# robdancer/SymbolicRegression.jl

Measured on AMD Instinct MI355X. Metric: tree-node x row evals/sec (whole node), 1k trees x 1M rows f32; % VALU peak, higher is better.
Workload: dtype f32; 1 GPU; C2 eval-only: 1024 random trees (size<=30) x 1M rows x 5 features Float32, fused L2 loss; ntrees_per_gpu=1024, rows=1000000, features=5, parallelism=single, trees_ok=808

## Files before the change

include/srhip.h:

```cpp
#ifndef SRHIP_H
#define SRHIP_H

#include <stdint.h>

#ifdef __cplusplus
extern "C" {
#endif

enum {
  SRHIP_OK = 0,
  SRHIP_ERR_INVALID = 1,
  SRHIP_ERR_UNSUPPORTED = 2,
  SRHIP_ERR_DEVICE = 3,
  SRHIP_ERR_NOMEM = 4
};

enum { SRHIP_F32 = 0, SRHIP_F64 = 1, SRHIP_I32 = 2 };

enum {
  SRHIP_OP_ADD = 1, SRHIP_OP_SUB = 2, SRHIP_OP_MUL = 3, SRHIP_OP_DIV = 4,
  SRHIP_OP_POW = 5,
  SRHIP_OP_GREATER = 6,
  SRHIP_OP_COND = 7,
  SRHIP_OP_LOGICAL_OR = 8,
// ... 152 lines not shown

typedef struct srhip_optim_options {
  int32_t iterations;
  int32_t nrestarts;
  uint64_t seed;
  double g_tol;
} srhip_optim_options;

int srhip_optimize_constants(srhip_ctx* ctx, const srhip_dataset* ds, srhip_program* prog,
                             const srhip_loss* loss, const int64_t* idx, int64_t nidx,
                             const srhip_optim_options* opt, double* out_loss,
                             uint8_t* out_improved, int64_t* out_fcalls);
int srhip_optimize_constants_starts(srhip_ctx* ctx, const srhip_dataset* ds, srhip_program* prog,
                                    const srhip_loss* loss, const int64_t* idx, int64_t nidx,
                                    const srhip_optim_options* opt, const double* starts_in,
                                    double* starts_out, double* out_loss, uint8_t* out_improved,
                                    int64_t* out_fcalls);

int srhip_eval_loss_grad_rowsets(srhip_ctx* ctx, const srhip_dataset* ds, srhip_program* prog,
                                 const srhip_loss* loss, const int64_t* row_offsets ,
                                 const int64_t* rows, double* out_loss, double* out_grad,
                                 uint8_t* out_ok);

int srhip_optimize_constants_rowsets(srhip_ctx* ctx, const srhip_dataset* ds, srhip_program* prog,
                                     const srhip_loss* loss, const int64_t* row_offsets ,
                                     const int64_t* rows, const srhip_optim_options* opt,
                                     const uint64_t* tree_seeds ,
                                     const double* starts_in , double* starts_out ,
                                     double* out_loss, uint8_t* out_improved, int64_t* out_fcalls);

double srhip_last_kernel_ms(const srhip_ctx* ctx);
int srhip_last_work(const srhip_ctx* ctx, int64_t out[4]);
int64_t srhip_hot_form_launches(const srhip_ctx* ctx);
int srhip_program_stats(const srhip_program* prog, int64_t* total_nodes, int64_t* total_opnodes,
                        int32_t* max_stack);
int srhip_program_derived(const srhip_program* prog, int32_t* count, uint32_t* spec, int32_t cap);
int32_t srhip_isa_handler_count(void);
int srhip_isa_handler_name(uint32_t h, char* buf, int32_t cap);
int srhip_isa_handler_ok(uint32_t h, int dtype);
int srhip_program_handlers(const srhip_program* prog, int32_t tree, int32_t derived, uint32_t* out, int32_t cap,
                           int32_t* count);
int srhip_code_cache_stats(int64_t* hits, int64_t* misses, int64_t* inserts);
int srhip_tail_share_parts(int32_t blocks, int32_t units, int32_t nshares, int32_t share, int32_t* out);

typedef struct srhip_batcher srhip_batcher;
int srhip_batcher_create(srhip_ctx* ctx, const srhip_dataset* ds, const srhip_operators* ops,
                         const srhip_loss* loss, int32_t max_batch, int32_t max_wait_us,
                         srhip_batcher** out);
int srhip_batcher_set_clients(srhip_batcher* b, int32_t nclients);
int srhip_batcher_submit(srhip_batcher* b, const srhip_node* nodes, int64_t nnodes,
                         const int64_t* idx, int64_t nidx, uint64_t* ticket);
int srhip_batcher_wait(srhip_batcher* b, uint64_t ticket, double* out_loss, uint8_t* out_ok);
int srhip_batcher_eval(srhip_batcher* b, const srhip_node* nodes, int64_t nnodes,
                       const int64_t* idx, int64_t nidx, double* out_loss, uint8_t* out_ok);
int srhip_batcher_stats(const srhip_batcher* b, int64_t* nrequests, int64_t* nlaunches,
                        int64_t* max_batch_seen);
int srhip_batcher_timing(const srhip_batcher* b, double* busy_ms, double* kernel_ms);
void srhip_batcher_destroy(srhip_batcher* b);

#ifdef __cplusplus
}
#endif
#endif
```

symbolicregression.jl_amd/csrc/srhip_eval_impl.h:

```cpp
#pragma once
#include <hip/hip_runtime.h>
#include <stdint.h>

#include <algorithm>
#include <type_traits>

#include "srhip_isa.h"
#include "srhip_kernels.h"
#include "srhip_ops.h"

#define UNR _Pragma("unroll")
#ifdef SRHIP_KDEBUG
#define KDBG(...) do { if (blockIdx.x == 0 && blockIdx.y == 0 && threadIdx.x == 0) printf(__VA_ARGS__); } while (0)
#else
#define KDBG(...) do { } while (0)
#endif
#ifdef SRHIP_KTRACE
#define KMARK(slot, val)                                                                       \
  do {                                                                                         \
    if (p.dbg && blockIdx.x == 0 && blockIdx.y == 0 && threadIdx.x == 0)                      \
      __hip_atomic_store(p.dbg + (slot), (int32_t)(val), __ATOMIC_RELAXED, __HIP_MEMORY_SCOPE_SYSTEM); \
  } while (0)
#else
#define KMARK(slot, val) do { } while (0)
// ... 1398 lines not shown
        UNR for (int o = 32; o > 0; o >>= 1) {
          if (MODE == MODE_LOSS) s += __shfl_xor(s, o);
          if constexpr (!kIsInt<T>) {
            if constexpr (sizeof(T) == 4) m = __builtin_elementwise_maximum(m, __shfl_xor(m, o));
            else m += __shfl_xor(m, o);
          }
        }
        if (lane == 0) {
          if (MODE == MODE_LOSS && p.fused_loss) reinterpret_cast<LAccT<T>*>(p.fused_loss)[tree] = s;
          if (p.fused_chk) reinterpret_cast<CT*>(p.fused_chk)[tree] = m;
          if (p.fused_rows) p.fused_rows[tree] = rows_done;
        }
      }
    }
    KMARK(8 + wave, 13);
    int claim = 0;
    if (lane == 0) claim = atomicAdd(&next_tree, 1);
    cl = __builtin_amdgcn_readfirstlane(claim);
  }
  KMARK(8 + wave, 14);
}

template <typename T, int R, int K, int MODE, bool XLDS, int FORM = FORM_GENERAL>
__global__ __launch_bounds__(64 * eval_waves(R, K)) void eval_kernel(EvalArgs p) {
  extern __shared__ __attribute__((aligned(16))) unsigned char smem[];
  constexpr bool HOT = FORM == FORM_HOT;
  KMARK(0, 1);
  if constexpr (!HOT)
    if (p.debug_stop == 1) return;
  __shared__ int claimed;
  if constexpr (MODE == MODE_PRECISE) {
    if (p.dev_count && p.grid_interleave && __builtin_amdgcn_readfirstlane(*p.dev_count) <= (int)blockIdx.y) return;
  }
  if (!HOT && p.tile_claims && !p.persistent) {
    if (p.zero_ctr && blockIdx.x == 0 && blockIdx.y == 0 && threadIdx.x == 0)
      __hip_atomic_store(p.zero_ctr, 0, __ATOMIC_RELAXED, __HIP_MEMORY_SCOPE_AGENT);
    const int gs = p.grid_interleave ? (int)blockIdx.y : 0, gst = p.grid_interleave ? (int)gridDim.y : 1;
    const int nz = p.grid_interleave ? (p.ntrees - gs + gst - 1) / gst : 0;
    for (int i = threadIdx.x; i < nz; i += blockDim.x) {
      const int64_t at = (int64_t)blockIdx.x * p.ntrees + gs + (int64_t)i * gst;
      if (p.slab_chk) __hip_atomic_store(reinterpret_cast<uint32_t*>(p.slab_chk) + at, 0u, __ATOMIC_RELAXED, __HIP_MEMORY_SCOPE_AGENT);
      if (p.slab_rows) __hip_atomic_store(p.slab_rows + at, 0, __ATOMIC_RELAXED, __HIP_MEMORY_SCOPE_AGENT);
    }
    __builtin_amdgcn_fence(__ATOMIC_RELEASE, "workgroup");
  }
  const int nfull = p.nrb - p.block0 - p.tail_blocks;
  const int nitems = nfull + (p.tail_blocks > 0 ? p.tail_shares : 0);
  int items = 0;
  int next_block = 0, next_units = 0;
  for (int it = 0;; ++it) {
    int rb, gy = 0, gslice = 0, gstride = 1, gw = 1;
    if ((HOT || p.persistent) && next_units > 0) {
      rb = next_block;
      gstride = p.tail_slices;
      gw = next_units;
      next_units = 0;
    } else if (HOT || p.persistent) {
      if (threadIdx.x == 0) claimed = atomicAdd(p.block_ctr, 1);
      __syncthreads();
      const int item = __builtin_amdgcn_readfirstlane(claimed);
      if (item >= nitems) {
        if (threadIdx.x == 0 && items > 0) atomicAdd(p.block_ctr + 1, items);
        if (threadIdx.x == 0 && item == nitems + (int)gridDim.x - 1)
          __hip_atomic_store(p.block_ctr, 0, __ATOMIC_RELAXED, __HIP_MEMORY_SCOPE_AGENT);
        break;
      }
      ++items;
      rb = p.block0 + item;
      if (item >= nfull) {
        TailPart part[2];
        const int nparts = tail_share_parts(p.tail_blocks, p.tail_slices, p.tail_shares, item - nfull, part);
        if (nparts == 0) {
          __syncthreads();
          continue;
        }
        rb = p.block0 + nfull + part[0].block;
        gslice = part[0].u0;
        gstride = p.tail_slices;
        gw = part[0].u1 - part[0].u0;
        if (nparts == 2) {
          next_block = rb + 1;
          next_units = part[1].u1;
        }
      }
    } else {
      rb = blockIdx.x + it * (int)gridDim.x;
      if (it > 0 && (!p.block_stride || rb >= p.nrb)) break;
      if (p.grid_interleave) {
        gslice = blockIdx.y;
        gstride = gridDim.y;
      } else {
        gy = blockIdx.y;
      }
    }
    eval_block<T, R, K, MODE, XLDS, FORM>(p, smem, rb, gy, gslice, gstride, gw);
    if (!HOT && !p.persistent && !p.block_stride) break;
    __syncthreads();
  }
}

template <typename T, int R, int K, int MODE, bool XLDS, int FORM = FORM_GENERAL>
inline hipError_t launch_eval_t(const EvalArgs& a, dim3 grid, size_t lds, hipStream_t s) {
  auto kern = eval_kernel<T, R, K, MODE, XLDS, FORM>;
  if (lds > 65536) {
    hipError_t e = hipFuncSetAttribute((const void*)kern, hipFuncAttributeMaxDynamicSharedMemorySize, (int)lds);
    if (e != hipSuccess) return e;
  }
  const int waves = a.wg_waves > 0 ? std::min(a.wg_waves, eval_waves(R, K)) : eval_waves(R, K);
  hipLaunchKernelGGL(kern, grid, dim3(64 * waves), lds, s, a);
  return hipGetLastError();
}

template <typename T, int R, int MODE, bool XLDS>
inline hipError_t launch_eval_k(const EvalArgs& a, int K, dim3 grid, size_t lds, hipStream_t s) {
  if (K <= 2) return launch_eval_t<T, R, 2, MODE, XLDS>(a, grid, lds, s);
  if (K <= 4) return launch_eval_t<T, R, 4, MODE, XLDS>(a, grid, lds, s);
  return launch_eval_t<T, R, 8, MODE, XLDS>(a, grid, lds, s);
}

template <typename T, int R, int MODE>
inline hipError_t launch_eval_mode(const EvalArgs& a, int K, bool xlds, dim3 grid, size_t lds, hipStream_t s) {
  if constexpr (MODE == MODE_PRECISE) {
    (void)K;
    (void)xlds;
    return launch_eval_t<T, R, K_MAX, MODE_PRECISE, false>(a, grid, lds, s);
  } else {
    return xlds ? launch_eval_k<T, R, MODE, true>(a, K, grid, lds, s) : launch_eval_k<T, R, MODE, false>(a, K, grid, lds, s);
  }
// ... 4 lines not shown
```

symbolicregression.jl_amd/csrc/srhip_host.cpp:

```cpp
#include <hip/hip_runtime.h>
#include <math.h>
#include <stdarg.h>
#include <stdint.h>
#include <stdio.h>
#include <stdlib.h>
#include <string.h>
#include <unistd.h>
#include <sys/resource.h>
#include <sys/syscall.h>

#include <algorithm>
#include <atomic>
#include <chrono>
#include <condition_variable>
#include <functional>
#include <memory>
#include <map>
#include <mutex>
#include <numeric>
#include <string>
#include <thread>
#include <type_traits>
#include <unordered_map>
#include <vector>

#include "../../include/srhip.h"
#include "srhip_internal.h"
#include "srhip_isa.h"
#include "srhip_kernels.h"
#include "srhip_ops.h"

using namespace srhip;

static bool env_flag(const char* name);

static thread_local std::string g_err;

int srhip::fail(int code, const char* fmt, ...) {
  char buf[1024];
  va_list ap;
  va_start(ap, fmt);
  vsnprintf(buf, sizeof(buf), fmt, ap);
  va_end(ap);
  g_err = buf;
  return code;
}
const char* srhip::last_error() { return g_err.c_str(); }

static thread_local std::chrono::steady_clock::time_point g_wait_begin, g_wait_done, g_tail_done;
extern "C" char** environ;
const char* srhip::env_get(const char* name) {
  struct Ent {
    const char* name;
    const char* val;
  };
  static thread_local uint64_t sig = 0;
  static thread_local std::vector<Ent> cache;
  uint64_t h = 1469598103934665603ull ^ (uint64_t)(uintptr_t)environ;
  for (char** e = environ; e && *e; ++e) h = (h ^ (uint64_t)(uintptr_t)*e) * 1099511628211ull;
  if (h != sig) {
    cache.clear();
    sig = h;
  }
// ... 1902 lines not shown
  {
    std::lock_guard<std::mutex> g(P->ord_mu);
    if (P->upload_pending || P->ord_key[0] != L.groups || P->ord_key[1] != L.tpg || P->ord_key[2] != (int)use_d ||
        P->ord_goff != goff || (persistent && P->ord_recs < 0)) {
      std::vector<int32_t>& order = P->ord_host;
      order = make_order(*P, live, goff, use_d);
      order.insert(order.end(), goff.begin(), goff.end());
      P->ord_recs = persistent ? append_slot_records(*P, order, nl, use_d) : -1;
      if (P->upload_pending) {
        const size_t base = P->blob_off[6], bytes = order.size() * sizeof(int32_t);
        P->blob.resize(base + bytes);
        memcpy(P->blob.data() + base, order.data(), bytes);
        HIP_TRY(P->d_prog.ensure(base + bytes));
        HIP_TRY(hipMemcpyAsync(P->d_prog.p, P->blob.data(), base + bytes, hipMemcpyHostToDevice, ctx->stream));
        set_prog_pointers(*P);
        P->upload_pending = false;
        P->ord_dev = (const uint8_t*)P->d_prog.p + base;
      } else {
        HIP_TRY(P->d_order.ensure(order.size() * sizeof(int32_t)));
        HIP_TRY(hipMemcpyAsync(P->d_order.p, order.data(), order.size() * sizeof(int32_t), hipMemcpyHostToDevice,
                               ctx->stream));
        P->ord_dev = P->d_order.p;
      }
      P->ord_key[0] = L.groups;
      P->ord_key[1] = L.tpg;
      P->ord_key[2] = (int)use_d;
      P->ord_goff = goff;
    }
    d_order = P->ord_dev;
    rec_at = P->ord_recs;
  }
  const int nch = (int)((v.m + loss_chunk(dtype) - 1) / loss_chunk(dtype));
  const int cpb = L.rb_rows / loss_chunk(dtype);
  HIP_TRY(ctx->slab_loss.ensure((size_t)nl * L.nrb * cpb * 8));
  HIP_TRY(ctx->slab_chk.ensure((size_t)nl * L.nrb * 8));
  HIP_TRY(rs->h_loss.ensure((size_t)nt * 8, hipHostMallocCoherent));
  HIP_TRY(rs->h_chk.ensure((size_t)nt * 8, hipHostMallocCoherent));
  HIP_TRY(rs->h_rows.ensure((size_t)(nt + 1) * 8, hipHostMallocCoherent));
  EvalArgs a{};
  a.code = use_d ? P->dcode_dev : P->code_dev;
  a.prog_off = use_d ? P->doff_dev : P->off_dev;
  a.order = (const int32_t*)d_order;
  a.nd = use_d ? nd : 0;
  a.dspec = use_d ? P->dspec_dev : nullptr;
  a.dmask = use_d ? P->dmask_dev : nullptr;
  if (dtype == SRHIP_F32) {
    if (!P->sbound_dev || P->sbound.size() != 4 * (size_t)P->ntrees)
      return fail(SRHIP_ERR_INVALID, "Float32 program without its +/- bounds");
    J.fbound = feature_bound(v, ds->nfeat);
  }
  a.X = v.X;
  a.y = v.y;
  a.w = weighted ? v.w : nullptr;
  a.slab_loss = ctx->slab_loss.p;
  a.slab_chk = ctx->slab_chk.p;
  a.ld = v.ld;
  a.nvalid = v.m;
  a.ntrees = nl;
  a.nfeat = P->maxfeat;
  a.rb_rows = L.rb_rows;
  a.nrb = L.nrb;
  a.nch = nch;
  a.cpb = cpb;
  a.trees_per_group = L.tpg;
  a.group_off = (const int32_t*)d_order + nl;
  a.loss_kind = loss ? loss->kind : 0;
  a.loss_p0 = loss ? loss->p0 : 0.0;
  a.weighted = weighted ? 1 : 0;
  a.has_y = mode == MODE_LOSS ? 1 : 0;
  a.max_steps = use_d ? P->dmax_len : P->max_len;
  a.debug_stop = debug_stop();
  if (small) a.wg_waves = (int)live.size();
  const char* nofuse = env_get("SRHIP_NO_FUSED_REDUCE");
  if (L.nrb == 1 && !sd && !(nofuse && *nofuse && *nofuse != '0')) {
    a.fused = 1;
    a.fused_loss = mode == MODE_LOSS ? rs->h_loss.p : nullptr;
    a.fused_chk = dtype == SRHIP_I32 ? nullptr : rs->h_chk.p;
    a.fused_rows = (int64_t*)rs->h_rows.p;
  } else {
    HIP_TRY(ctx->slab_rows.ensure((size_t)nl * L.nrb * sizeof(int32_t)));
    a.slab_rows = (int32_t*)ctx->slab_rows.p;
  }
  const bool devp = dp && !a.fused && dtype != SRHIP_I32 && !env_flag("SRHIP_NO_DEVICE_PRECISE");
  int ucap = std::max(1, std::min(DEV_PRECISE_MAX, env_int("SRHIP_PRECISE_LIST", DEV_PRECISE_MAX)));
  if (devp) {
    const int rc = ensure_dev_precise(ctx, P, v, &ucap, rs);
    if (rc) return rc;
  }
  a.early_exit = mode == MODE_LOSS && early_exit_on() ? 1 : 0;
  if (a.early_exit) {
    const int rc = next_fail_epoch(ctx, nl, &a.fail_flag, &a.epoch);
    if (rc) return rc;
  }
  if (trace_on()) {
    HIP_TRY(ctx->h_dbg.ensure(64 * sizeof(int32_t), hipHostMallocCoherent));
    memset(ctx->h_dbg.p, 0xff, 64 * sizeof(int32_t));
    a.dbg = (int32_t*)ctx->h_dbg.p;
  }
  DevBuf& pred = J.pred;
  if (mode == MODE_PRED) {
    HIP_TRY(pred.ensure((size_t)nt * v.m * es));
    a.out_pred = pred.p;
  }
  dim3 grid(L.nrb, (unsigned)goff.size() - 1);
  const bool probe_zeroes = probe_blocks > 0 && !env_flag("SRHIP_PROBE_TREE_CLAIMS");
  if (persistent && (!ctx->block_ctr.p || (ctx->block_ctr_dirty && !probe_zeroes))) {
    HIP_TRY(ctx->block_ctr.ensure(2 * sizeof(int32_t)));
    HIP_TRY(hipMemsetAsync(ctx->block_ctr.p, 0, 2 * sizeof(int32_t), ctx->stream));
    ctx->block_ctr_dirty = false;
  }
  if (persistent) ctx->block_ctr_dirty = true;
  if (sd) HIP_TRY(hipMemsetAsync(sd->d_loss, 0, sd->zero_bytes, ctx->stream));
  HIP_TRY(hipEventRecord(rs->ev0, ctx->stream));
  if (persistent) {
    if (probe_blocks > 0) {
      EvalArgs q = a;
      q.group_off = nullptr;
      q.trees_per_group = eval_waves(R, K);
      q.grid_interleave = 1;
      if (probe_zeroes) {
        q.tile_claims = 1;
        q.zero_ctr = (int32_t*)ctx->block_ctr.p;
      }
      q.code = P->code_dev;
      q.prog_off = P->off_dev;
      q.max_steps = P->max_len;
      q.nd = 0;
      q.dspec = nullptr;
      q.dmask = nullptr;
      const size_t qlds = (size_t)(P->maxfeat + 1 + (weighted ? 1 : 0)) * L.rb_rows * es + 16;
      const dim3 pgrid(probe_blocks, (unsigned)((nl + q.trees_per_group - 1) / q.trees_per_group));
      HIP_TRY(launch_eval(dtype, q, R, K, mode, true, pgrid, qlds, ctx->stream));
    }
    a.persistent = 1;
    a.block0 = probe_blocks;
    a.block_ctr = (int32_t*)ctx->block_ctr.p;
    if (const int seed = env_int("SRHIP_DEBUG_BLOCK_CTR", 0)) {
      const int32_t h = (int32_t)seed;
      HIP_TRY(hipMemcpyAsync(ctx->block_ctr.p, &h, sizeof(h), hipMemcpyHostToDevice, ctx->stream));
      HIP_TRY(hipStreamSynchronize(ctx->stream));
    }
    const int nmain = L.nrb - probe_blocks;
    constexpr int TAIL_UNITS = 128;
    const int wgs_cap = std::max(1, std::min(env_int("SRHIP_PERSISTENT_WGS", ctx->num_cu), ctx->num_cu));
    const int units_env = env_int("SRHIP_TAIL_SLICES", 0);
    const int units = units_env > 1 ? std::min(units_env, 128) : TAIL_UNITS;
    int wgs = std::max(1, std::min(nmain, wgs_cap));
    a.tail_slices = 1;
    a.tail_blocks = 0;
    a.tail_shares = 0;
    if (env_int("SRHIP_TAIL_BALANCE", 1) != 0 && nmain % wgs_cap != 0) {
      const int lb = nmain % wgs_cap;
      const int nshares = wgs_cap * (env_int("SRHIP_TAIL_SHARE_ROUNDS", 1) == 2 ? 2 : 1);
      if ((int64_t)nl * lb >= (int64_t)eval_waves(R, K) * nshares &&
          (int64_t)lb * units * nshares < ((int64_t)1 << 31)) {
        wgs = wgs_cap;
        a.tail_slices = units;
        a.tail_blocks = lb;
        a.tail_shares = nshares;
      }
    }
    J.expect_items = nmain - a.tail_blocks + a.tail_shares;
    if (R == R_F32_WIDE && K == 2 && rec_at >= 0 && !a.fused && a.slab_rows && !a.dbg && a.debug_stop == 0 &&
        a.loss_kind >= 0 && a.loss_kind < 256 && (int64_t)nl * L.nrb * cpb < ((int64_t)1 << 31) && !env_flag("SRHIP_NO_HOT_FORM"))
      a.recs = (const SlotRec*)((const int32_t*)d_order + rec_at);
    HIP_TRY(launch_eval(dtype, a, R, K, mode, true, dim3(wgs, 1), L.lds, ctx->stream));
    if (a.recs) ++ctx->hot_launches;
  } else {
    HIP_TRY(launch_eval(dtype, a, R, K, mode, L.xlds, grid, L.lds, ctx->stream));
  }
  HIP_TRY(hipEventRecord(rs->ev1, ctx->stream));
  J.launched = true;
  J.persistent = persistent;
  J.devp = devp;
  if (trace_on()) {
// ... 585 lines not shown

int srhip_ctx_synchronize(srhip_ctx* ctx) {
  if (!ctx) return fail(SRHIP_ERR_INVALID, "null ctx");
  HIP_TRY(hipStreamSynchronize(ctx->stream));
  return SRHIP_OK;
}

int srhip_dataset_create(srhip_ctx* ctx, int dtype, const void* X, int64_t nfeat, int64_t n, int64_t sf, int64_t sr,
                         const void* y, const void* w, srhip_dataset** out) {
  if (!ctx || !out) return fail(SRHIP_ERR_INVALID, "null argument");
  *out = nullptr;
  if (dtype != SRHIP_F32 && dtype != SRHIP_F64 && dtype != SRHIP_I32) return fail(SRHIP_ERR_UNSUPPORTED, "dtype %d", dtype);
  if (n <= 0) return fail(SRHIP_ERR_INVALID, "dataset needs n >= 1 rows");
  if (nfeat < 0 || nfeat > 65535) return fail(SRHIP_ERR_INVALID, "nfeatures %lld out of range", (long long)nfeat);
  if (nfeat > 0 && !X) return fail(SRHIP_ERR_INVALID, "null X");
  if (dtype == SRHIP_I32 && w) return fail(SRHIP_ERR_UNSUPPORTED, "weights on Int32 datasets");
  HIP_TRY(hipSetDevice(ctx->device));
  std::unique_ptr<srhip_dataset> d(new srhip_dataset());
  static std::atomic<uint64_t> g_ds_serial{0};
  d->serial = ++g_ds_serial;
  d->ctx = ctx;
  d->device = ctx->device;
  d->dtype = dtype;
  d->nfeat = nfeat;
  d->n = n;
  d->ld = (n + ROW_ALIGN - 1) / ROW_ALIGN * ROW_ALIGN;
  d->has_y = y != nullptr;
  d->weighted = w != nullptr;
  const size_t es = dtype_size(dtype);
  const size_t colb = (size_t)d->ld * es;
  HIP_TRY(d->X.ensure(std::max<size_t>(1, (size_t)nfeat) * colb));
  HostBuf stage;
  HIP_TRY(stage.ensure(colb));
  for (int64_t f = 0; f < nfeat; ++f) {
    if (dtype == SRHIP_F64) pack_column<uint64_t>(X, f, n, sf, sr, d->ld, (uint64_t*)stage.p);
    else pack_column<uint32_t>(X, f, n, sf, sr, d->ld, (uint32_t*)stage.p);
    HIP_TRY(hipMemcpy((char*)d->X.p + f * colb, stage.p, colb, hipMemcpyHostToDevice));
  }
  if (y) {
    HIP_TRY(d->y.ensure(colb));
    if (dtype == SRHIP_F64) pack_column<uint64_t>(y, 0, n, 0, 1, d->ld, (uint64_t*)stage.p);
    else pack_column<uint32_t>(y, 0, n, 0, 1, d->ld, (uint32_t*)stage.p);
    HIP_TRY(hipMemcpy(d->y.p, stage.p, colb, hipMemcpyHostToDevice));
  }
  if (w) {
    HIP_TRY(d->w.ensure(colb));
    double s = 0.0;
    if (dtype == SRHIP_F64) {
      double* st = (double*)stage.p;
      for (int64_t j = 0; j < d->ld; ++j) st[j] = j < n ? ((const double*)w)[j] : 0.0;
      for (int64_t j = 0; j < n; ++j) s += st[j];
    } else {
      float* st = (float*)stage.p;
      for (int64_t j = 0; j < d->ld; ++j) st[j] = j < n ? ((const float*)w)[j] : 0.0f;
      for (int64_t j = 0; j < n; ++j) s += st[j];
    }
    d->sum_w = s;
    HIP_TRY(hipMemcpy(d->w.p, stage.p, colb, hipMemcpyHostToDevice));
  }
  d->hstats.assign(std::max<int64_t>(1, nfeat), FeatStat{0.0, 0});
  if (dtype != SRHIP_I32 && nfeat > 0) {
    HIP_TRY(d->stats.ensure(feature_stats_scratch(nfeat) * sizeof(FeatStat)));
    HIP_TRY(launch_feature_stats(dtype, d->X.p, d->ld, n, (int)nfeat, (FeatStat*)d->stats.p, ctx->stream));
    HIP_TRY(hipMemcpyAsync(d->hstats.data(), d->stats.p, (size_t)nfeat * sizeof(FeatStat), hipMemcpyDeviceToHost,
                           ctx->stream));
    HIP_TRY(hipStreamSynchronize(ctx->stream));
  }
  *out = d.release();
  return SRHIP_OK;
}
// ... 425 lines not shown
  if (hipEventElapsedTime(&ms, ctx->last_ev0, ctx->last_ev1) != hipSuccess) return -1.0;
  return (double)ms;
}

int srhip_code_cache_stats(int64_t* hits, int64_t* misses, int64_t* inserts) {
  if (hits) *hits = g_cache_hits.load();
  if (misses) *misses = g_cache_misses.load();
  if (inserts) *inserts = g_cache_inserts.load();
  return SRHIP_OK;
}

int srhip_tail_share_parts(int32_t blocks, int32_t units, int32_t nshares, int32_t share, int32_t* out) {
  if (!out || blocks < 1 || units < 1 || nshares < blocks || share < 0 || share >= nshares ||
      (int64_t)blocks * units * nshares >= ((int64_t)1 << 31))
    return -1;
  TailPart part[2];
  const int n = tail_share_parts(blocks, units, nshares, share, part);
  for (int i = 0; i < n; ++i) {
    out[3 * i] = part[i].block;
    out[3 * i + 1] = part[i].u0;
    out[3 * i + 2] = part[i].u1;
  }
  return n;
}

int srhip_last_work(const srhip_ctx* ctx, int64_t* out) {
  if (!ctx || !out) return fail(SRHIP_ERR_INVALID, "null argument");
  for (int i = 0; i < 4; ++i) out[i] = ctx->work[i];
  return SRHIP_OK;
}

int64_t srhip_hot_form_launches(const srhip_ctx* ctx) { return ctx ? ctx->hot_launches : -1; }

int srhip_program_stats(const srhip_program* P, int64_t* total_nodes, int64_t* total_opnodes, int32_t* max_stack) {
  if (!P) return fail(SRHIP_ERR_INVALID, "null program");
  if (total_nodes) *total_nodes = P->total_nodes;
  if (total_opnodes) *total_opnodes = P->total_ops;
  if (max_stack) *max_stack = P->kmax;
  return SRHIP_OK;
}

int srhip_program_derived(const srhip_program* P, int32_t* count, uint32_t* spec, int32_t cap) {
  if (!P) return fail(SRHIP_ERR_INVALID, "null program");
  if (count) *count = (int32_t)P->dspec.size();
  for (int32_t d = 0; spec && d < cap && d < (int32_t)P->dspec.size(); ++d) spec[d] = P->dspec[d];
  return SRHIP_OK;
}

int32_t srhip_isa_handler_count(void) { return (int32_t)H_COUNT; }

int srhip_isa_handler_name(uint32_t h, char* buf, int32_t cap) {
  if (!buf || cap < 1) return fail(SRHIP_ERR_INVALID, "null or empty name buffer");
  if (h >= H_COUNT) return fail(SRHIP_ERR_INVALID, "handler id %u out of range (< %u)", h, H_COUNT);
  static const char* const spec_names[] = {
#define X_(n, f) #n,
      SRHIP_SPEC_BINOPS(X_)
#undef X_
  };
  static const char* const heavy_names[] = {
#define X_(n, f) #n,
      SRHIP_HEAVY_BINOPS(X_)
#undef X_
  };
  static const char* const un_names[] = {
#define X_(n, f) #f,
      SRHIP_UNOPS(X_)
// ... 56 lines not shown
```

symbolicregression.jl_amd/csrc/srhip_internal.h:

```cpp
#pragma once
#include <hip/hip_runtime.h>
#include <math.h>
#include <stdarg.h>
#include <stdint.h>
#include <stdio.h>
#include <stdlib.h>
#include <string.h>

#include <chrono>
#include <functional>
#include <mutex>
#include <string>
#include <vector>

#include "../../include/srhip.h"
#include "srhip_isa.h"
#include "srhip_kernels.h"

namespace srhip {

int fail(int code, const char* fmt, ...);
const char* last_error();

inline bool trace_on() {
// ... 121 lines not shown

struct srhip_ctx {
  int device = 0;
  hipStream_t stream = nullptr;
  hipEvent_t ev0 = nullptr, ev1 = nullptr;
  hipEvent_t last_ev0 = nullptr, last_ev1 = nullptr;
  srhip::ResultSet rs[srhip::RESULT_SETS];
  hipEvent_t ev_sync = nullptr;
  hipStream_t up_stream = nullptr;
  bool timed = false;
  int num_cu = 256;
  int lds_max = 160 * 1024;
  srhip::DevBuf slab_loss, slab_chk, slab_prec, order_prec;
  srhip::DevBuf vX, vy, vw, vidx, vstats;
  srhip::DevBuf g_chunks, g_slab, g_red;
  srhip::DevBuf g_rs_packed, g_rs_meta;
  srhip::DevBuf g_xd;
  uint64_t g_xd_serial = 0;
  int64_t g_xd_ld = 0;
  int g_xd_dtype = -1, g_xd_base = -1;
  std::vector<uint32_t> g_xd_spec;
  srhip::HostBuf h_gchunks[2], h_gred[2];
  srhip::HostBuf h_gpatch, h_gspec;
  srhip::HostBuf h_stats, h_prec, h_plist, h_dbg;
  srhip::HostBuf h_rowsets;
  srhip::DevBuf fail_flag;
  int32_t epoch = 0;
  srhip::DevBuf block_ctr;
  bool block_ctr_dirty = false;
  srhip::DevBuf slab_rows;
  srhip::DevBuf d_ulist;
  int64_t work[4] = {0, 0, 0, 0};
  int64_t hot_launches = 0;
  std::vector<srhip_ctx*> aux;
  std::mutex aux_mu;
};

struct srhip_dataset {
  srhip_ctx* ctx = nullptr;
  int device = 0;
  int dtype = SRHIP_F32;
  int64_t nfeat = 0, n = 0, ld = 0;
  bool has_y = false, weighted = false;
  double sum_w = 0.0;
  srhip::DevBuf X, y, w, stats;
  std::vector<srhip::FeatStat> hstats;
  uint64_t serial = 0;
};

struct srhip_program {
  srhip_ctx* ctx = nullptr;
  int device = -1;
  int dtype = SRHIP_F32;
  int32_t ntrees = 0;
  std::vector<srhip_node> nodes;
  std::vector<int64_t> offsets;
  std::vector<int32_t> binops, unaops;
  std::vector<srhip::TreeInfo> info;
  std::vector<srhip::TreeDecide> dec;
  std::vector<srhip::Ins> code;
  std::vector<int32_t> prog_off;
  int32_t kmax = 0, max_ops = 0, max_len = 0;
  int64_t total_nodes = 0, total_ops = 0;
  int32_t maxfeat = 0;
  mutable srhip::PoolBuf d_prog;
  mutable std::vector<uint8_t> blob;
  mutable bool upload_pending = false;
  mutable int32_t und_hint = 0;
  mutable size_t blob_off[7] = {0, 0, 0, 0, 0, 0, 0};
  mutable const srhip::Ins* code_dev = nullptr;
  mutable const int32_t* off_dev = nullptr;
  std::vector<uint32_t> dspec;
  std::vector<uint64_t> dmask;
  std::vector<srhip::Ins> dcode;
  std::vector<int32_t> dprog_off;
  std::vector<double> dcost;
  int32_t dkmax = 0, dmax_len = 0;
  mutable const srhip::Ins* dcode_dev = nullptr;
  mutable const int32_t* doff_dev = nullptr;
  mutable const uint32_t* dspec_dev = nullptr;
// ... 123 lines not shown
```

symbolicregression.jl_amd/csrc/srhip_kernels.h:

```cpp
#pragma once
#include <hip/hip_runtime.h>
#include <stdint.h>

#include "srhip_isa.h"
#include "srhip_tail_shares.h"

namespace srhip {

#ifndef SRHIP_EVAL_WAVES
#define SRHIP_EVAL_WAVES 8
#endif
constexpr int EVAL_WAVES = SRHIP_EVAL_WAVES;
constexpr int EVAL_WAVES_WIDE = 16;
constexpr int eval_waves(int R, int K) { return (R == 16 && K <= 2) ? EVAL_WAVES_WIDE : EVAL_WAVES; }
constexpr int EVAL_WAVES_MAX = EVAL_WAVES_WIDE > EVAL_WAVES ? EVAL_WAVES_WIDE : EVAL_WAVES;
#ifndef SRHIP_R_F32
#define SRHIP_R_F32 8
#endif
constexpr int R_F32 = SRHIP_R_F32;
constexpr int R_F64 = 4;
constexpr int R_F32_WIDE = 16;
constexpr int64_t WIDE_MIN_ROWS = 4096;
constexpr int ROW_ALIGN = 4096;
constexpr int MODE_LOSS = 0, MODE_PRED = 1, MODE_PRECISE = 2;
// ... 41 lines not shown
  int32_t loss_kind;
  double loss_p0;
  int32_t weighted;
  int32_t prec_stride;
  int32_t has_y;
  int32_t max_steps;
  int32_t debug_stop;
  int32_t nd;
  const uint32_t* dspec;
  const uint64_t* dmask;
  int32_t* dbg;
  int32_t early_exit;
  int32_t epoch;
  int32_t* fail_flag;
  int32_t fused;
  void* fused_loss;
  void* fused_chk;
  int32_t persistent;
  int32_t block0;
  int32_t tail_blocks;
  int32_t tail_slices;
  int32_t tail_shares;
  int32_t grid_interleave;
  int32_t tile_claims;
  int32_t block_stride;
  int32_t* block_ctr;
  int32_t* zero_ctr;
  const int32_t* dev_count;
  int32_t wg_waves;
  int32_t prec_assign;
  int32_t* slab_rows;
  int64_t* fused_rows;
  const SlotRec* recs;
};

int rows_per_lane(int dtype);
int pick_rows_per_lane(int dtype, int K, int mode, int64_t m);
hipError_t launch_eval(int dtype, const EvalArgs& a, int R, int K, int mode, bool xlds, dim3 grid, size_t lds,
                       hipStream_t s);
struct UndecidedList {
  int32_t* ulist = nullptr;
  int32_t umax = 0;
  double rows = 0.0;
  const float* sbound = nullptr;
  float fbound = 0.0f;
};
__host__ __device__ inline float skip_bound_apply(float M, const float* sb, float F) {
  if (!(sb[0] > 0.0f || sb[1] > 0.0f || sb[2] > 0.0f) || !(M - M == 0.0f)) return M;
  const double fb = sb[1] > 0.0f ? (double)sb[1] * (double)F : 0.0;
  const double bd = (double)sb[0] * (double)M + (fb + (double)sb[2]);
  const double mb = bd > (double)M ? bd : (double)M;
  return mb < (double)__FLT_MAX__ ? (float)mb : __FLT_MAX__;
}
hipError_t launch_reduce(int dtype, const void* slab_loss, int nch, int cpb, const void* slab_chk, int nrb, int nslots,
                         const int32_t* order, void* out_loss, void* out_chk, hipStream_t s,
                         const int32_t* slab_rows = nullptr, int64_t* out_rows = nullptr,
                         const UndecidedList& ul = UndecidedList(), bool chk_inf = false,
                         int32_t* items_done = nullptr, int64_t* out_items = nullptr);
hipError_t launch_precise_reduce(const double* slab, int nrb, int stride, int32_t* ulist, int umax, int groups, int done_slot,
                                 int32_t* out_list, double* out, hipStream_t s);
hipError_t launch_gather(int dtype, const void* X, const void* y, const void* w, int64_t ld_src, int nfeat,
                         const int64_t* idx, int64_t m, int64_t ld_dst, void* Xd, void* yd, void* wd, hipStream_t s);
hipError_t launch_feature_stats(int dtype, const void* X, int64_t ld, int64_t m, int nfeat, FeatStat* out,
                                hipStream_t s);

struct RowsetArgs {
// ... 15 lines not shown
```

symbolicregression.jl_amd/srhip/_lib.py:

```python
from __future__ import annotations

import ctypes
import os
import threading

import numpy as np

_PKG_DIR = os.path.dirname(os.path.abspath(__file__))
LIB_PATH = os.environ.get(
    "SRHIP_LIB", os.path.join(os.path.dirname(_PKG_DIR), "build", "libsrhip.so")
)

OK, ERR_INVALID, ERR_UNSUPPORTED, ERR_DEVICE, ERR_NOMEM = 0, 1, 2, 3, 4
COMM_ID_BYTES = 128
REDUCE_SUM, REDUCE_MAX = 0, 1
F32, F64, I32 = 0, 1, 2

OP = dict(
    ADD=1, SUB=2, MUL=3, DIV=4, POW=5, GREATER=6, COND=7, LOGICAL_OR=8, LOGICAL_AND=9,
    MAX=10, MIN=11, MOD=12, ATAN2=13,
    NEG=32, SQUARE=33, CUBE=34, ABS=35, RELU=36, COS=37, SIN=38, TAN=39, EXP=40, LOG=41,
    LOG2=42, LOG10=43, LOG1P=44, SQRT=45, ACOSH=46, ATANH_CLIP=47, SINH=48, COSH=49, TANH=50,
    ASIN=51, ACOS=52, ATAN=53, ASINH=54, ERF=55, ERFC=56, GAMMA=57, ROUND=58, FLOOR=59,
    CEIL=60, SIGN=61, EXP2=62, EXPM1=63, CBRT=64,
# ... 67 lines not shown
    "srhip_eval_loss_grad": (ctypes.c_int, [_vp, _vp, _vp, ctypes.POINTER(Loss), _vp, _i64, _vp, _vp, _vp]),
    "srhip_eval_grad_predict": (ctypes.c_int, [_vp, _vp, _vp, _i32, _i32, _vp, _i64, _vp, _vp, _vp]),
    "srhip_optimize_constants": (ctypes.c_int, [_vp, _vp, _vp, ctypes.POINTER(Loss), _vp, _i64,
                                                ctypes.POINTER(OptimOptions), _vp, _vp, _vp]),
    "srhip_optimize_constants_starts": (ctypes.c_int, [_vp, _vp, _vp, ctypes.POINTER(Loss), _vp, _i64,
                                                       ctypes.POINTER(OptimOptions), _vp, _vp, _vp, _vp, _vp]),
    "srhip_eval_loss_grad_rowsets": (ctypes.c_int, [_vp, _vp, _vp, ctypes.POINTER(Loss), _vp, _vp, _vp, _vp, _vp]),
    "srhip_optimize_constants_rowsets": (ctypes.c_int, [_vp, _vp, _vp, ctypes.POINTER(Loss), _vp, _vp,
                                                        ctypes.POINTER(OptimOptions), _vp, _vp, _vp, _vp, _vp, _vp]),
    "srhip_batcher_create": (ctypes.c_int, [_vp, _vp, ctypes.POINTER(Operators), ctypes.POINTER(Loss), _i32, _i32,
                                            ctypes.POINTER(_vp)]),
    "srhip_batcher_set_clients": (ctypes.c_int, [_vp, _i32]),
    "srhip_batcher_submit": (ctypes.c_int, [_vp, _vp, _i64, _vp, _i64, ctypes.POINTER(ctypes.c_uint64)]),
    "srhip_batcher_wait": (ctypes.c_int, [_vp, ctypes.c_uint64, ctypes.POINTER(_dbl), ctypes.POINTER(ctypes.c_uint8)]),
    "srhip_batcher_eval": (ctypes.c_int, [_vp, _vp, _i64, _vp, _i64, ctypes.POINTER(_dbl),
                                          ctypes.POINTER(ctypes.c_uint8)]),
    "srhip_batcher_stats": (ctypes.c_int, [_vp, ctypes.POINTER(_i64), ctypes.POINTER(_i64), ctypes.POINTER(_i64)]),
    "srhip_batcher_timing": (ctypes.c_int, [_vp, ctypes.POINTER(ctypes.c_double), ctypes.POINTER(ctypes.c_double)]),
    "srhip_batcher_destroy": (None, [_vp]),
    "srhip_comm_unique_id": (ctypes.c_int, [_vp]),
    "srhip_comm_create": (ctypes.c_int, [_vp, _vp, _i32, _i32, ctypes.POINTER(_vp)]),
    "srhip_comm_destroy": (None, [_vp]),
    "srhip_comm_size": (ctypes.c_int, [_vp, ctypes.POINTER(_i32), ctypes.POINTER(_i32)]),
    "srhip_comm_stats": (ctypes.c_int, [_vp, ctypes.POINTER(ctypes.c_double), ctypes.POINTER(ctypes.c_double),
                                        ctypes.POINTER(ctypes.c_int64)]),
    "srhip_comm_allreduce_f64": (ctypes.c_int, [_vp, _vp, _i64, _i32]),
    "srhip_comm_allgather": (ctypes.c_int, [_vp, _vp, _i64, _vp]),
    "srhip_comm_migrate_start": (ctypes.c_int, [_vp, _vp, _vp, _i32, _vp, _i32, _i32]),
    "srhip_comm_migrate_wait": (ctypes.c_int, [_vp, _vp, _vp, _vp, _vp]),
    "srhip_eval_loss_sharded": (ctypes.c_int, [_vp, _vp, _vp, _vp, ctypes.POINTER(Loss), _vp, _i64, _vp, _vp]),
    "srhip_last_kernel_ms": (_dbl, [_vp]),
    "srhip_last_work": (ctypes.c_int, [_vp, ctypes.POINTER(_i64)]),
    "srhip_hot_form_launches": (ctypes.c_int64, [_vp]),
    "srhip_program_stats": (ctypes.c_int, [_vp, ctypes.POINTER(_i64), ctypes.POINTER(_i64),
                                           ctypes.POINTER(_i32)]),
    "srhip_program_derived": (ctypes.c_int, [_vp, ctypes.POINTER(_i32), _vp, _i32]),
    "srhip_isa_handler_count": (_i32, []),
    "srhip_isa_handler_name": (ctypes.c_int, [ctypes.c_uint32, ctypes.c_char_p, _i32]),
    "srhip_isa_handler_ok": (ctypes.c_int, [ctypes.c_uint32, ctypes.c_int]),
    "srhip_program_handlers": (ctypes.c_int, [_vp, _i32, _i32, _vp, _i32, ctypes.POINTER(_i32)]),
    "srhip_code_cache_stats": (ctypes.c_int, [ctypes.POINTER(_i64), ctypes.POINTER(_i64), ctypes.POINTER(_i64)]),
    "srhip_tail_share_parts": (ctypes.c_int, [_i32, _i32, _i32, _i32, _vp]),
}

_lib = None
_lock = threading.Lock()


def load() -> ctypes.CDLL:
    global _lib
    with _lock:
        if _lib is not None:
            return _lib
        if not os.path.exists(LIB_PATH):
            raise SrhipError(ERR_DEVICE, f"{LIB_PATH} not built: run `make -C symbolicregression.jl_amd` "
                                         "(or __graft_entry__.build()); there is no CPU fallback")
        lib = ctypes.CDLL(LIB_PATH)
        for name, (res, args) in SIGNATURES.items():
            try:
                fn = getattr(lib, name)
            except AttributeError:
                continue
            fn.restype = res
            fn.argtypes = args
        _lib = lib
        return lib
# ... 25 lines not shown
```

symbolicregression.jl_amd/srhip/device.py:

```python
from __future__ import annotations

import ctypes
import threading

import numpy as np

from . import _lib
from ._lib import check, ptr


class Context:
    def __init__(self, device: int = 0):
        lib = _lib.load()
        h = ctypes.c_void_p()
        check(lib.srhip_ctx_create(int(device), ctypes.byref(h)))
        self.handle = h
        self.device = int(device)
        self._lib = lib

    def synchronize(self):
        check(self._lib.srhip_ctx_synchronize(self.handle))

    def last_kernel_ms(self) -> float:
        return float(self._lib.srhip_last_kernel_ms(self.handle))

    def last_work(self) -> dict:
        out = (ctypes.c_int64 * 4)()
        check(self._lib.srhip_last_work(self.handle, out))
        return {"node_rows": int(out[0]), "nominal_node_rows": int(out[1]), "opnode_rows": int(out[2]),
                "tree_rows": int(out[3])}

    def hot_form_launches(self) -> int:
        return int(self._lib.srhip_hot_form_launches(self.handle))

    def close(self):
        if self.handle:
            self._lib.srhip_ctx_destroy(self.handle)
            self.handle = None

    def __del__(self):
        try:
            self.close()
        except Exception:
            pass


_tls = threading.local()


def get_context(device: int = 0) -> Context:
    cache = getattr(_tls, "ctxs", None)
    if cache is None:
        cache = _tls.ctxs = {}
    ctx = cache.get(device)
    if ctx is None:
        ctx = cache[device] = Context(device)
    return ctx


def isa_handler_count() -> int:
    return int(_lib.load().srhip_isa_handler_count())


def isa_handler_name(h: int) -> str:
    buf = ctypes.create_string_buffer(32)
    check(_lib.load().srhip_isa_handler_name(int(h), buf, 32))
# ... 9 lines not shown

def device_count() -> int:
    try:
        return int(_lib.load().srhip_device_count())
    except _lib.SrhipError:
        return 0


class DeviceDataset:

    def __init__(self, ctx: Context, X: np.ndarray, y=None, weights=None):
        X = np.asarray(X)
        if X.ndim != 2:
            raise ValueError("X must be (nfeatures, n)")
        self.dtype = X.dtype
        code = _lib.dtype_code(X.dtype)
        nfeat, n = X.shape
        es = X.itemsize
        sf, sr = X.strides[0] // es, X.strides[1] // es
        if X.strides[0] % es or X.strides[1] % es:
            X = np.ascontiguousarray(X)
            sf, sr = n, 1
        yv = None if y is None else np.ascontiguousarray(y, dtype=X.dtype)
        wv = None if weights is None else np.ascontiguousarray(weights, dtype=X.dtype)
        h = ctypes.c_void_p()
        check(_lib.load().srhip_dataset_create(ctx.handle, code, ptr(X), nfeat, n, sf, sr, ptr(yv), ptr(wv),
                                               ctypes.byref(h)))
        self.handle = h
        self.ctx = ctx
        self.nfeatures = nfeat
        self.n = n
        self.weighted = weights is not None

    def close(self):
        if self.handle:
            _lib.load().srhip_dataset_destroy(self.handle)
            self.handle = None

    def __del__(self):
        try:
            self.close()
        except Exception:
            pass


def pack_rowsets(idxs, ntrees=None):
    sets = [np.ascontiguousarray(i, dtype=np.int64).reshape(-1) for i in idxs]
    if ntrees is not None and len(sets) != ntrees:
        raise ValueError(f"{len(sets)} row subsets for {ntrees} trees")
    for t, i in enumerate(sets):
        if i.size == 0:
            raise ValueError(f"row subset of tree {t} is empty")
    offsets = np.zeros(len(sets) + 1, dtype=np.int64)
    np.cumsum([i.size for i in sets], out=offsets[1:])
    rows = np.concatenate(sets) if sets else np.zeros(0, dtype=np.int64)
    return offsets, rows


class Program:

    def __init__(self, ctx: Context | None, nodes: np.ndarray, offsets: np.ndarray, options, dtype):
        self.ctx = ctx
        self.nodes = np.ascontiguousarray(nodes)
        self.offsets = np.ascontiguousarray(offsets, dtype=np.int64)
        self.ntrees = len(self.offsets) - 1
        self.options = options
# ... 294 lines not shown
```

Before: 11430 billion node-row evals/s.

## Add sentinel-row probe block to detect non-finite trees early

```diff
diff --git a/include/srhip.h b/include/srhip.h
--- a/include/srhip.h
+++ b/include/srhip.h
@@ -208,6 +208,8 @@
 double srhip_last_kernel_ms(const srhip_ctx* ctx);
 int srhip_last_work(const srhip_ctx* ctx, int64_t out[4]);
 int64_t srhip_hot_form_launches(const srhip_ctx* ctx);
+int64_t srhip_sentinel_launches(const srhip_ctx* ctx);
+int64_t srhip_dataset_sentinel_rows(const srhip_dataset* ds, int64_t* out, int64_t cap);
 int srhip_program_stats(const srhip_program* prog, int64_t* total_nodes, int64_t* total_opnodes,
                         int32_t* max_stack);
 int srhip_program_derived(const srhip_program* prog, int32_t* count, uint32_t* spec, int32_t cap);
diff --git a/symbolicregression.jl_amd/csrc/srhip_eval_impl.h b/symbolicregression.jl_amd/csrc/srhip_eval_impl.h
--- a/symbolicregression.jl_amd/csrc/srhip_eval_impl.h
+++ b/symbolicregression.jl_amd/csrc/srhip_eval_impl.h
@@ -1454,15 +1454,34 @@
   if constexpr (MODE == MODE_PRECISE) {
     if (p.dev_count && p.grid_interleave && __builtin_amdgcn_readfirstlane(*p.dev_count) <= (int)blockIdx.y) return;
   }
+  constexpr bool SENT = !HOT && MODE == MODE_LOSS && XLDS && !kIsInt<T> && sizeof(T) == 4 && R == R_F32_WIDE;
+  [[maybe_unused]] EvalArgs ps = p;
+  [[maybe_unused]] bool sent = false;
+  if constexpr (SENT) {
+    sent = p.sent_rows > 0 && !p.persistent && blockIdx.x == gridDim.x - 1;
+    if (sent) {
+      const int64_t row = (int64_t)p.nrb * p.ntrees;
+      ps.X = p.sent_X;
+      ps.y = p.sent_y;
+      ps.w = p.sent_w;
+      ps.ld = p.sent_ld;
+      ps.nvalid = p.sent_rows;
+      ps.slab_loss = reinterpret_cast<LAccT<T>*>(p.slab_loss) + row * p.cpb;
+      ps.slab_chk = reinterpret_cast<typename Chk<T>::type*>(p.slab_chk) + row;
+      ps.slab_rows = p.slab_rows ? p.slab_rows + row : nullptr;
+    }
+  }
+  const EvalArgs& pe = SENT ? ps : p;
+  const int grid_rb = sent ? 0 : (int)blockIdx.x;
   if (!HOT && p.tile_claims && !p.persistent) {
     if (p.zero_ctr && blockIdx.x == 0 && blockIdx.y == 0 && threadIdx.x == 0)
       __hip_atomic_store(p.zero_ctr, 0, __ATOMIC_RELAXED, __HIP_MEMORY_SCOPE_AGENT);
     const int gs = p.grid_interleave ? (int)blockIdx.y : 0, gst = p.grid_interleave ? (int)gridDim.y : 1;
     const int nz = p.grid_interleave ? (p.ntrees - gs + gst - 1) / gst : 0;
     for (int i = threadIdx.x; i < nz; i += blockDim.x) {
-      const int64_t at = (int64_t)blockIdx.x * p.ntrees + gs + (int64_t)i * gst;
-      if (p.slab_chk) __hip_atomic_store(reinterpret_cast<uint32_t*>(p.slab_chk) + at, 0u, __ATOMIC_RELAXED, __HIP_MEMORY_SCOPE_AGENT);
-      if (p.slab_rows) __hip_atomic_store(p.slab_rows + at, 0, __ATOMIC_RELAXED, __HIP_MEMORY_SCOPE_AGENT);
+      const int64_t at = (int64_t)grid_rb * p.ntrees + gs + (int64_t)i * gst;
+      if (pe.slab_chk) __hip_atomic_store(reinterpret_cast<uint32_t*>(pe.slab_chk) + at, 0u, __ATOMIC_RELAXED, __HIP_MEMORY_SCOPE_AGENT);
+      if (pe.slab_rows) __hip_atomic_store(pe.slab_rows + at, 0, __ATOMIC_RELAXED, __HIP_MEMORY_SCOPE_AGENT);
     }
     __builtin_amdgcn_fence(__ATOMIC_RELEASE, "workgroup");
   }
@@ -1506,7 +1525,7 @@
         }
       }
     } else {
-      rb = blockIdx.x + it * (int)gridDim.x;
+      rb = grid_rb + it * (int)gridDim.x;
       if (it > 0 && (!p.block_stride || rb >= p.nrb)) break;
       if (p.grid_interleave) {
         gslice = blockIdx.y;
@@ -1515,7 +1534,7 @@
         gy = blockIdx.y;
       }
     }
-    eval_block<T, R, K, MODE, XLDS, FORM>(p, smem, rb, gy, gslice, gstride, gw);
+    eval_block<T, R, K, MODE, XLDS, FORM>(pe, smem, rb, gy, gslice, gstride, gw);
     if (!HOT && !p.persistent && !p.block_stride) break;
     __syncthreads();
   }
diff --git a/symbolicregression.jl_amd/csrc/srhip_host.cpp b/symbolicregression.jl_amd/csrc/srhip_host.cpp
--- a/symbolicregression.jl_amd/csrc/srhip_host.cpp
+++ b/symbolicregression.jl_amd/csrc/srhip_host.cpp
@@ -29,6 +29,7 @@
 #include "srhip_isa.h"
 #include "srhip_kernels.h"
 #include "srhip_ops.h"
+#include "srhip_sentinel.h"
 
 using namespace srhip;
 
@@ -1997,8 +1998,14 @@
   }
   const int nch = (int)((v.m + loss_chunk(dtype) - 1) / loss_chunk(dtype));
   const int cpb = L.rb_rows / loss_chunk(dtype);
-  HIP_TRY(ctx->slab_loss.ensure((size_t)nl * L.nrb * cpb * 8));
-  HIP_TRY(ctx->slab_chk.ensure((size_t)nl * L.nrb * 8));
+  bool finite_x = v.stats != nullptr;
+  for (int64_t f = 0; finite_x && f < nf; ++f) finite_x = v.stats[f].nonfinite == 0;
+  const bool sentinel = probe_blocks >= 2 && mode == MODE_LOSS && early_exit_on() && !ds->sent_idx.empty() &&
+                        v.X == ds->X.p && v.m == ds->n && (int64_t)ds->sent_idx.size() <= L.rb_rows &&
+                        L.rb_rows <= ds->sent_ld && finite_x && env_int("SRHIP_SENTINEL_ROWS", 1) != 0;
+  const size_t slab_nrb = (size_t)L.nrb + (sentinel ? 1 : 0);
+  HIP_TRY(ctx->slab_loss.ensure((size_t)nl * slab_nrb * cpb * 8));
+  HIP_TRY(ctx->slab_chk.ensure((size_t)nl * slab_nrb * 8));
   HIP_TRY(rs->h_loss.ensure((size_t)nt * 8, hipHostMallocCoherent));
   HIP_TRY(rs->h_chk.ensure((size_t)nt * 8, hipHostMallocCoherent));
   HIP_TRY(rs->h_rows.ensure((size_t)(nt + 1) * 8, hipHostMallocCoherent));
@@ -2043,7 +2050,7 @@
     a.fused_chk = dtype == SRHIP_I32 ? nullptr : rs->h_chk.p;
     a.fused_rows = (int64_t*)rs->h_rows.p;
   } else {
-    HIP_TRY(ctx->slab_rows.ensure((size_t)nl * L.nrb * sizeof(int32_t)));
+    HIP_TRY(ctx->slab_rows.ensure((size_t)nl * slab_nrb * sizeof(int32_t)));
     a.slab_rows = (int32_t*)ctx->slab_rows.p;
   }
   const bool devp = dp && !a.fused && dtype != SRHIP_I32 && !env_flag("SRHIP_NO_DEVICE_PRECISE");
@@ -2094,18 +2101,27 @@
       q.dspec = nullptr;
       q.dmask = nullptr;
       const size_t qlds = (size_t)(P->maxfeat + 1 + (weighted ? 1 : 0)) * L.rb_rows * es + 16;
+      if (sentinel) {
+        const uint8_t* const sb = (const uint8_t*)ds->sent.p;
+        q.sent_X = sb;
+        q.sent_y = sb + (size_t)(nf * ds->sent_ld) * es;
+        q.sent_w = weighted ? sb + (size_t)((nf + 1) * ds->sent_ld) * es : nullptr;
+        q.sent_ld = (int32_t)ds->sent_ld;
+        q.sent_rows = (int32_t)ds->sent_idx.size();
+      }
       const dim3 pgrid(probe_blocks, (unsigned)((nl + q.trees_per_group - 1) / q.trees_per_group));
       HIP_TRY(launch_eval(dtype, q, R, K, mode, true, pgrid, qlds, ctx->stream));
+      if (sentinel) ++ctx->sentinel_launches;
     }
     a.persistent = 1;
-    a.block0 = probe_blocks;
+    a.block0 = probe_blocks - (sentinel ? 1 : 0);
     a.block_ctr = (int32_t*)ctx->block_ctr.p;
     if (const int seed = env_int("SRHIP_DEBUG_BLOCK_CTR", 0)) {
       const int32_t h = (int32_t)seed;
       HIP_TRY(hipMemcpyAsync(ctx->block_ctr.p, &h, sizeof(h), hipMemcpyHostToDevice, ctx->stream));
       HIP_TRY(hipStreamSynchronize(ctx->stream));
     }
-    const int nmain = L.nrb - probe_blocks;
+    const int nmain = L.nrb - a.block0;
     constexpr int TAIL_UNITS = 128;
     const int wgs_cap = std::max(1, std::min(env_int("SRHIP_PERSISTENT_WGS", ctx->num_cu), ctx->num_cu));
     const int units_env = env_int("SRHIP_TAIL_SLICES", 0);
@@ -2757,10 +2773,32 @@
   HIP_TRY(d->X.ensure(std::max<size_t>(1, (size_t)nfeat) * colb));
   HostBuf stage;
   HIP_TRY(stage.ensure(colb));
+  const int sent_k = dtype == SRHIP_F32 && y && (n + SENT_BLOCK_ROWS - 1) / SENT_BLOCK_ROWS >= 64 ? sentinel_k(nfeat) : 0;
+  std::vector<int64_t> sent_rows;
   for (int64_t f = 0; f < nfeat; ++f) {
     if (dtype == SRHIP_F64) pack_column<uint64_t>(X, f, n, sf, sr, d->ld, (uint64_t*)stage.p);
     else pack_column<uint32_t>(X, f, n, sf, sr, d->ld, (uint32_t*)stage.p);
     HIP_TRY(hipMemcpy((char*)d->X.p + f * colb, stage.p, colb, hipMemcpyHostToDevice));
+    if (sent_k > 0) sentinel_scan_column((const float*)stage.p, n, sent_k, sent_rows);
+  }
+  if (sent_k > 0) {
+    sentinel_merge(sent_rows);
+    const int64_t ns = (int64_t)sent_rows.size(), sld = SENT_BLOCK_ROWS;
+    if (ns > 0 && ns <= sld) {
+      const int64_t ncol = nfeat + 1 + (w ? 1 : 0);
+      std::vector<uint32_t> img((size_t)(ncol * sld));
+      for (int64_t c = 0; c < ncol; ++c) {
+        const uint32_t* src = c < nfeat ? (const uint32_t*)X + c * sf : (const uint32_t*)(c == nfeat ? y : w);
+        const int64_t step = c < nfeat ? sr : 1;
+        uint32_t* dst = img.data() + c * sld;
+        for (int64_t i = 0; i < ns; ++i) dst[i] = src[sent_rows[i] * step];
+        for (int64_t i = ns; i < sld; ++i) dst[i] = c > nfeat ? 0u : dst[ns - 1];
+      }
+      HIP_TRY(d->sent.ensure(img.size() * sizeof(uint32_t)));
+      HIP_TRY(hipMemcpy(d->sent.p, img.data(), img.size() * sizeof(uint32_t), hipMemcpyHostToDevice));
+      d->sent_ld = sld;
+      d->sent_idx = std::move(sent_rows);
+    }
   }
   if (y) {
     HIP_TRY(d->y.ensure(colb));
@@ -3252,6 +3290,15 @@
 
 int64_t srhip_hot_form_launches(const srhip_ctx* ctx) { return ctx ? ctx->hot_launches : -1; }
 
+int64_t srhip_sentinel_launches(const srhip_ctx* ctx) { return ctx ? ctx->sentinel_launches : -1; }
+
+int64_t srhip_dataset_sentinel_rows(const srhip_dataset* ds, int64_t* out, int64_t cap) {
+  if (!ds) return -1;
+  const int64_t ns = (int64_t)ds->sent_idx.size();
+  for (int64_t i = 0; out && i < std::min(ns, cap); ++i) out[i] = ds->sent_idx[i];
+  return ns;
+}
+
 int srhip_program_stats(const srhip_program* P, int64_t* total_nodes, int64_t* total_opnodes, int32_t* max_stack) {
   if (!P) return fail(SRHIP_ERR_INVALID, "null program");
   if (total_nodes) *total_nodes = P->total_nodes;
diff --git a/symbolicregression.jl_amd/csrc/srhip_internal.h b/symbolicregression.jl_amd/csrc/srhip_internal.h
--- a/symbolicregression.jl_amd/csrc/srhip_internal.h
+++ b/symbolicregression.jl_amd/csrc/srhip_internal.h
@@ -177,6 +177,7 @@
   srhip::DevBuf d_ulist;
   int64_t work[4] = {0, 0, 0, 0};
   int64_t hot_launches = 0;
+  int64_t sentinel_launches = 0;
   std::vector<srhip_ctx*> aux;
   std::mutex aux_mu;
 };
@@ -191,6 +192,9 @@
   srhip::DevBuf X, y, w, stats;
   std::vector<srhip::FeatStat> hstats;
   uint64_t serial = 0;
+  srhip::DevBuf sent;
+  int64_t sent_ld = 0;
+  std::vector<int64_t> sent_idx;
 };
 
 struct srhip_program {
diff --git a/symbolicregression.jl_amd/csrc/srhip_kernels.h b/symbolicregression.jl_amd/csrc/srhip_kernels.h
--- a/symbolicregression.jl_amd/csrc/srhip_kernels.h
+++ b/symbolicregression.jl_amd/csrc/srhip_kernels.h
@@ -97,6 +97,11 @@
   int32_t* slab_rows;
   int64_t* fused_rows;
   const SlotRec* recs;
+  const void* sent_X;
+  const void* sent_y;
+  const void* sent_w;
+  int32_t sent_ld;
+  int32_t sent_rows;
 };
 
 int rows_per_lane(int dtype);
diff --git a/symbolicregression.jl_amd/csrc/srhip_sentinel.h b/symbolicregression.jl_amd/csrc/srhip_sentinel.h
--- /dev/null
+++ b/symbolicregression.jl_amd/csrc/srhip_sentinel.h
@@ -0,0 +1,83 @@
+#pragma once
+#include <stdint.h>
+
+#include <algorithm>
+#include <vector>
+
+namespace srhip {
+
+constexpr int SENT_BLOCK_ROWS = 2048;
+constexpr int SENT_K_MAX = 128;
+
+inline int sentinel_k(int64_t nfeat) {
+  return nfeat > 0 ? (int)std::min<int64_t>(SENT_K_MAX, SENT_BLOCK_ROWS / (3 * nfeat)) : 0;
+}
+
+template <typename T>
+struct SentinelHeap {
+  struct E {
+    T key;
+    int64_t row;
+    bool operator<(const E& o) const { return key < o.key || (key == o.key && row < o.row); }
+  };
+  std::vector<E> h;
+  size_t k = 0;
+  explicit SentinelHeap(int k_) : k((size_t)k_) { h.reserve(k); }
+  void offer(T key, int64_t row) {
+    if (h.size() < k) {
+      h.push_back(E{key, row});
+      std::push_heap(h.begin(), h.end());
+    } else if (key < h.front().key) {
+      std::pop_heap(h.begin(), h.end());
+      h.back() = E{key, row};
+      std::push_heap(h.begin(), h.end());
+    }
+  }
+  void drop_worst() {
+    std::pop_heap(h.begin(), h.end());
+    h.pop_back();
+  }
+};
+
+inline void sentinel_scan_column(const float* col, int64_t n, int k, std::vector<int64_t>& rows) {
+  if (k <= 0 || n <= 0) return;
+  using T = float;
+  SentinelHeap<T> big(k), small(k), zero(k);
+  int64_t bad = -1;
+  constexpr int64_t CHUNK = 256;
+  for (int64_t c0 = 0; c0 < n; c0 += CHUNK) {
+    const int64_t c1 = std::min(n, c0 + CHUNK);
+    if (zero.h.size() == (size_t)k) {
+      const T tb = -big.h.front().key, ts = small.h.front().key, tz = zero.h.front().key;
+      int any = 0;
+      for (int64_t j = c0; j < c1; ++j) {
+        const T v = col[j], av = __builtin_fabsf(v);
+        any |= (int)(v > tb) | (int)(v < ts) | (int)(av < tz) | (int)!(av < __builtin_inff());
+      }
+      if (!any) continue;
+    }
+    for (int64_t j = c0; j < c1; ++j) {
+      const T v = col[j];
+      if (!(v - v == T(0))) {
+        if (bad < 0) bad = j;
+        continue;
+      }
+      big.offer(-v, j);
+      small.offer(v, j);
+      zero.offer(v < T(0) ? -v : v, j);
+    }
+  }
+  if (bad >= 0) {
+    if (zero.h.size() == (size_t)k) zero.drop_worst();
+    rows.push_back(bad);
+  }
+  for (const SentinelHeap<T>* s : {&big, &small, &zero})
+    for (const auto& e : s->h) rows.push_back(e.row);
+}
+
+inline void sentinel_merge(std::vector<int64_t>& rows) {
+  std::sort(rows.begin(), rows.end());
+  rows.erase(std::unique(rows.begin(), rows.end()), rows.end());
+}
+
+}
diff --git a/symbolicregression.jl_amd/srhip/_lib.py b/symbolicregression.jl_amd/srhip/_lib.py
--- a/symbolicregression.jl_amd/srhip/_lib.py
+++ b/symbolicregression.jl_amd/srhip/_lib.py
@@ -123,6 +123,8 @@
     "srhip_last_kernel_ms": (_dbl, [_vp]),
     "srhip_last_work": (ctypes.c_int, [_vp, ctypes.POINTER(_i64)]),
     "srhip_hot_form_launches": (ctypes.c_int64, [_vp]),
+    "srhip_sentinel_launches": (ctypes.c_int64, [_vp]),
+    "srhip_dataset_sentinel_rows": (ctypes.c_int64, [_vp, _vp, _i64]),
     "srhip_program_stats": (ctypes.c_int, [_vp, ctypes.POINTER(_i64), ctypes.POINTER(_i64),
                                            ctypes.POINTER(_i32)]),
     "srhip_program_derived": (ctypes.c_int, [_vp, ctypes.POINTER(_i32), _vp, _i32]),
diff --git a/symbolicregression.jl_amd/srhip/device.py b/symbolicregression.jl_amd/srhip/device.py
--- a/symbolicregression.jl_amd/srhip/device.py
+++ b/symbolicregression.jl_amd/srhip/device.py
@@ -32,6 +32,9 @@
 
     def hot_form_launches(self) -> int:
         return int(self._lib.srhip_hot_form_launches(self.handle))
+
+    def sentinel_launches(self) -> int:
+        return int(self._lib.srhip_sentinel_launches(self.handle))
 
     def close(self):
         if self.handle:
@@ -107,6 +110,14 @@
         self.n = n
         self.weighted = weights is not None
 
+    def sentinel_rows(self) -> np.ndarray:
+        lib = _lib.load()
+        n = int(lib.srhip_dataset_sentinel_rows(self.handle, None, 0))
+        out = np.zeros(max(n, 0), np.int64)
+        if n > 0:
+            lib.srhip_dataset_sentinel_rows(self.handle, ptr(out), n)
+        return out
+
     def close(self):
         if self.handle:
             _lib.load().srhip_dataset_destroy(self.handle)
```

New measurement: 11260 billion node-row evals/s. -1.4%, worse.
